# DLR-RB/QUEASARS

Measured on AMD Instinct MI355X. Metric: circuit-evals/sec (EVQE population) at n qubits; achieved HBM GB/s vs roofline, higher is better.
Workload: dtype f64; 1 GPU; 20-qubit EVQE population=64 per GPU, 4 layers, random Ising Hamiltonian (210 terms), fp64 (BASELINE.json configs[1]); n_qubits=20, population_per_gpu=64, layers=4, pauli_terms=210, parallelism=1 GPU

## Files before the change

include/qsv.h:

```cpp
#ifndef QSV_H
#define QSV_H

#include <stddef.h>
#include <stdint.h>

#ifdef __cplusplus
extern "C" {
#endif

typedef struct qsv_handle qsv_t;

enum { QSV_OP_ID = 0, QSV_OP_U = 1, QSV_OP_CU3 = 2 };
enum { QSV_F64 = 0, QSV_F32 = 1 };
enum { QSV_NO_CONTROL = 0xFF };

enum {
    QSV_OK = 0,
    QSV_E_ARG = -1,
    QSV_E_DEVICE = -2,
    QSV_E_STATE = -3,
    QSV_E_UNSUPPORTED = -4
};

typedef struct qsv_op {
// ... 258 lines not shown
int qsv_set_option(qsv_t* h, const char* name, int value);

long long qsv_replayed_pushes(const qsv_t* h);

int qsv_set_profiling(qsv_t* h, int enabled);
int qsv_get_profile(const qsv_t* h, qsv_profile* out);

int qsv_bench_gate(qsv_t* h, int target, int control, double theta, double phi, double lambda, int reps,
                   double* out_ms_per_sweep);

int qsv_bench_ops(qsv_t* h, int n_ops, const qsv_op* ops, int reps, double* out_ms_per_rep, int* out_n_passes);

int qsv_plan_build(int n_qubits, int dtype, int n_ops, const qsv_op* ops, const qsv_plan_config* cfg,
                   uint32_t* out_words, size_t capacity_words, size_t* n_words);

int qsv_split_describe(int n_qubits, int n_ops, const qsv_op* ops, int max_side, uint64_t* mask_a, qsv_op* ops_a,
                       int capacity_a, int* n_ops_a, qsv_op* ops_b, int capacity_b, int* n_ops_b);

#define QSV_SPLIT_MAX_KEYS 8
int qsv_split_describe_reduced(int n_qubits, int n_ops, const qsv_op* ops, int max_side, uint64_t* mask_a, qsv_op* ops_a,
                               int capacity_a, int* n_ops_a, qsv_op* ops_b, int capacity_b, int* n_ops_b,
                               uint32_t* simulated_keys, uint32_t* final_keys, int* key_bits, int* qubits);

const char* qsv_version(void);

#ifdef __cplusplus
}
#endif
#endif
```

queasars_amd/_lib.py:

```python

from __future__ import annotations

import ctypes as C
import os
import threading
from pathlib import Path

import numpy as np

from queasars_amd import _build

QSV_OK, QSV_E_ARG, QSV_E_DEVICE, QSV_E_STATE, QSV_E_UNSUPPORTED = 0, -1, -2, -3, -4
QSV_F64, QSV_F32 = 0, 1


class QsvOp(C.Structure):
    _fields_ = [
        ("kind", C.c_uint8),
        ("target", C.c_uint8),
        ("control", C.c_uint8),
        ("flags", C.c_uint8),
        ("p_theta", C.c_int32),
        ("p_phi", C.c_int32),
        ("p_lambda", C.c_int32),
# ... 247 lines not shown
                                       C.POINTER(C.c_int32), C.POINTER(C.c_int32)]),
    "qsv_adjoint_gradient_circuits": (C.c_int, [_P, C.c_int, _P, _P, _P, _P, _P, _P, _P]),
    "qsv_adjoint_gradient_device": (C.c_int, [_P, C.c_int, _P, C.c_int, _P, _P, _P, _P, C.c_int, _P, _P]),
    "qsv_adjoint_stats": (C.c_int, [_P, C.POINTER(QsvAdjointStats)]),
    "qsv_observables_create": (C.c_int, [_P, C.c_int, _P, _P, _P, _P, _P, C.POINTER(C.c_int)]),
    "qsv_observables_destroy": (C.c_int, [_P, C.c_int]),
    "qsv_eval_observables": (C.c_int, [_P, C.c_int, C.c_int, _P, _P, _P, _P]),
    "qsv_set_option": (C.c_int, [_P, C.c_char_p, C.c_int]),
    "qsv_fitness_table_wait": (C.c_int, [C.c_void_p, C.c_int, C.c_void_p, C.c_int, C.c_int, C.c_int, C.c_int64, C.c_int]),
    "qsv_replayed_pushes": (C.c_longlong, [_P]),
    "qsv_set_profiling": (C.c_int, [_P, C.c_int]),
    "qsv_get_profile": (C.c_int, [_P, C.POINTER(QsvProfile)]),
    "qsv_bench_gate": (C.c_int, [_P, C.c_int, C.c_int, C.c_double, C.c_double, C.c_double, C.c_int, C.POINTER(C.c_double)]),
    "qsv_bench_ops": (C.c_int, [_P, C.c_int, _P, C.c_int, C.POINTER(C.c_double), C.POINTER(C.c_int)]),
    "qsv_split_describe": (
        C.c_int,
        [C.c_int, C.c_int, _P, C.c_int, C.POINTER(C.c_uint64), _P, C.c_int, C.POINTER(C.c_int), _P, C.c_int, C.POINTER(C.c_int)],
    ),
    "qsv_split_describe_reduced": (
        C.c_int,
        [C.c_int, C.c_int, _P, C.c_int, C.POINTER(C.c_uint64), _P, C.c_int, C.POINTER(C.c_int), _P, C.c_int, C.POINTER(C.c_int),
         _P, _P, _P, _P],
    ),
    "qsv_plan_build": (
        C.c_int,
        [C.c_int, C.c_int, C.c_int, _P, C.POINTER(QsvPlanConfig), _P, C.c_size_t, C.POINTER(C.c_size_t)],
    ),
}

_lock = threading.Lock()
_lib = None


class QsvLibraryError(RuntimeError):
    """libqsv is missing or could not be loaded.  There is deliberately no fallback."""


def library_path() -> Path:
    override = os.environ.get("QSV_LIBRARY")
    return Path(override) if override else _build.LIB_PATH


def load(build_if_missing: bool = True) -> C.CDLL:
    global _lib
    with _lock:
        if _lib is not None:
# ... 33 lines not shown
```

queasars_amd/csrc/qsv_api.hip:

```cpp
#include <hip/hip_runtime.h>
#include <immintrin.h>

#include <algorithm>
#include <atomic>
#include <chrono>
#include <cmath>
#include <cstdio>
#include <condition_variable>
#include <cstring>
#include <functional>
#include <memory>
#include <mutex>
#include <string>
#include <thread>
#include <unordered_map>
#include <vector>

#include "../../include/qsv.h"
#include "adjoint.hpp"
#include "gradient.hpp"
#include "value_cache.hpp"
#include "kernels.hpp"
#include "plan.hpp"
#include "split.hpp"
// ... 194 lines not shown
    DeviceBuffer d_factor_big_count;
    uint32_t stream_mode = 0;
    mutable std::mutex mu;
    std::atomic<std::thread::id> batch_owner{};

    int n_terms = 0;
    bool diagonal = false;
    bool has_diag_part = false;
    int n_groups = 0;
    DeviceBuffer d_z, d_cre, d_diag, d_term_partials, d_groups, d_term_odd;
    DeviceBuffer d_order, d_sorted;
    bool order_valid = false;
    int pauli_nb = 0;

    std::unordered_map<int, Circuit> circuits;
    int next_circuit_id = 1;
    std::unordered_map<int, PrefixState> prefixes;
    int next_prefix_id = 1;
    DeviceBuffer d_prefix;
    DeviceBuffer d_sdiag;
    size_t sdiag_used = 0;
    bool side_diag = true;
    bool final_controls = true;
    bool sides_r3 = true;
    size_t prefix_slots = 0;
    std::vector<uint32_t> prefix_free;
    size_t prefix_used = 0;
    std::unordered_map<std::string, int> inline_cache;
    std::unordered_map<int, ObservableSet> obs_sets;
    int next_obs_id = 1;
    DeviceBuffer d_obs_partials, d_obs_values;
    std::unique_ptr<WorkerPool> pool;
    std::mutex pool_mu;

    struct CoalesceRequest {
        int circuit_id = 0;
        const double* params = nullptr;
        int n_params = 0;
        double value = 0.0;
        int rc = QSV_OK;
        std::string err;
        bool done = false;
    };
    std::mutex cq_mu;
    std::condition_variable cq_cv;
    std::vector<CoalesceRequest*> cq;
// ... 397 lines not shown
    }
    out->n_params = n_params;
    out->ops.assign(ops, ops + n_ops);
    out->grad_terms.assign(size_t(n_params), 0);
    (void)gradient_plan(n_ops, ops, n_params, out->grad_terms.data());
    std::vector<AngleSource> angles;
    std::vector<GateIn> gates = gates_of(ops, n_ops, &angles);
    out->n_gates = int(gates.size());
    out->fold = fold;
    try {
        PlanConfig pc = h->cfg;
        pc.fold = pc.fold && fold;
        const bool state_needed = h->n_terms > 0 && !h->diagonal && !h->factor_enabled;
        if (h->split_enabled && !state_needed && pc.fold && h->n > h->geo.k && h->n <= 28) {
            const int side_tile = std::max(h->geo.k, std::min(h->geo.r + 9, int(kMaxTileBits)));
            std::vector<int> limits{h->geo.k};
            if (side_tile > h->geo.k && side_tile < h->n) limits.push_back(side_tile);
            for (int extra = 1; extra <= kSideExtraBits; ++extra) {
                const int limit = std::min(h->geo.k + extra, h->n - 1);
                if (limit > limits.back()) limits.push_back(limit);
            }
            SplitCircuits sc = find_split(h->n, gates, angles, limits, h->split_max_keys);
            if (sc.ok && std::max(sc.n_side[0], sc.n_side[1]) > kSideMaxOwnBits) sc.ok = false;
            if (sc.ok) {
                SplitInfo& sp = out->split;
                std::vector<uint32_t>& w = out->plan.words;
                bool fits = true;
                const bool r3_handle = h->sides_r3 && h->dtype == QSV_F64 && h->geo.k == 12 && h->geo.r == 4 && sc.n_keys <= 3;
                bool try_halves = r3_handle && sc.n_keys >= 1 && std::max(sc.n_side[0], sc.n_side[1]) + sc.n_keys == kFusedLdsRowsBits &&
                                  !getenv("QSV_NO_HALF_SIDES");
                const int most_virtual = std::max(sc.n_side[0], sc.n_side[1]) + sc.n_keys;
                bool try_r3 = try_halves || (r3_handle && (most_virtual <= 12 || (most_virtual == 13 && sc.n_keys >= 1)));
                const size_t words_before = w.size();
                for (bool planned = false; !planned;) {
                planned = true;
                for (int s = 0; s < 2 && fits && planned; ++s) {
                    PlanConfig side = pc;
                    sp.n_virtual[s] = sc.n_side[s] + sc.n_keys;
                    side.tile_bits = std::min(sp.n_virtual[s], side_tile);
                    side.reg_bits = try_r3 ? 3 : h->geo.r;
                    side.compact = false;
                    fits = side.tile_bits > side.reg_bits;
                    if (!fits) break;
                    if (sp.n_virtual[s] <= side.tile_bits) side.lane_bits = 0;
                    if (try_halves && sp.n_virtual[s] == kFusedLdsRowsBits) {
                        side.tile_bits = 12;
                        side.lane_bits = 0;
// ... 73 lines not shown
                    }
                    auto fill = [&](uint32_t* table, uint32_t entries, int first_bit) {
                        table[0] = table[1] = 0;
                        for (uint32_t v = 1; v < entries; ++v) {
                            const uint32_t low = v & (0u - v), rest = v ^ low;
                            const int q = first_bit + __builtin_ctz(low);
                            table[2 * v] = table[2 * rest] | (q < h->n ? colx[size_t(q)] : 0u);
                            table[2 * v + 1] = table[2 * rest + 1] | (q < h->n ? coly[size_t(q)] : 0u);
                        }
                    };
                    fill(blk + kSplitLaneTable, 64, 0);
                    fill(blk + kSplitWaveTable, 1u << wave_bits, 6);
                    fill(blk + kSplitChunkLow, 128, chunk0);
                    fill(blk + kSplitChunkHigh, 128, chunk0 + 7);
                    sp.n_keys = sc.n_keys;
                    sp.ok = true;
                    sp.fused = h->geo.r == 4 && h->geo.k == 12 && sp.n_keys <= 3 && ((sp.outer[0] == 0 && sp.outer[1] == 0) || sp.halves || (sp.side_r == 3 && sp.outer[0] <= 1 && sp.outer[1] <= 1)) &&
                               sp.stats[0].n_passes == 1 && sp.stats[1].n_passes == 1;
                    if (const char* env = getenv("QSV_FUSED_MAX_KEYS")) sp.fused = sp.fused && sp.n_keys <= atoi(env);
                    if (getenv("QSV_SPLIT_DEBUG"))
                        fprintf(stderr, "split: keys %d sides %d+%d virtual %d/%d tiles 2^%d/2^%d passes %d/%d fused %d\n", sp.n_keys, sc.n_side[0],
                                sc.n_side[1], sp.n_virtual[0], sp.n_virtual[1], sp.outer[0], sp.outer[1], sp.stats[0].n_passes,
                                sp.stats[1].n_passes, int(sp.fused));
                    if (sp.fused && h->final_controls) plan_reduced_sides(h, pc, sc, sx, out);
                } else {
                    w.resize(sp.off_side[0] ? sp.off_side[0] : w.size());
                    sp = SplitInfo{};
                }
            }
        }
        if (out->split.ok) {
            out->gates = std::move(gates);
            out->angles = std::move(angles);
        } else {
            const CircuitPlan p = build_ordinary_plan(h, gates, angles, pc);
            out->off_plan = uint32_t(out->plan.words.size());
            out->plan.words.insert(out->plan.words.end(), p.words.begin(), p.words.end());
            out->plan.stats = p.stats;
            out->has_plan = true;
        }
    } catch (const std::exception& e) {
        if (err) *err = std::string("plan: ") + e.what();
        return QSV_E_ARG;
    }
    return QSV_OK;
}

int ensure_plan(qsv_t* h, Circuit& c) {
    if (c.has_plan) return QSV_OK;
    try {
        PlanConfig pc = h->cfg;
// ... 1591 lines not shown
    if (const char* env = getenv("QSV_TILES_PER_BLOCK_LATER")) h->tiles_per_block_later = std::max(1, atoi(env));
    auto bail = [&](hipError_t err, const char* what) {
        std::string msg = std::string(what) + ": " + hipGetErrorString(err);
        qsv_destroy(h);
        return fail(nullptr, QSV_E_DEVICE, msg);
    };
    if ((e = hipStreamCreateWithFlags(&h->stream, hipStreamNonBlocking)) != hipSuccess) return bail(e, "hipStreamCreate");
    h->own_stream = true;
    if (const char* env = getenv("QSV_SPLIT")) h->split_enabled = atoi(env) != 0;
    if (const char* env = getenv("QSV_SPLIT_SAMPLE")) h->split_sampling = atoi(env) != 0;
    if (const char* env = getenv("QSV_FACTOR")) h->factor_enabled = atoi(env) != 0;
    if (getenv("QSV_NO_FUSED_FACTOR")) h->fused_factor = false;
    if (const char* env = getenv("QSV_CHAIN_STREAM")) h->chain_enabled = atoi(env) != 0;
    if (const char* env = getenv("QSV_POLL")) h->poll_results = atoi(env) != 0;
    if (const char* env = getenv("QSV_REPEAT")) h->repeat_enabled = atoi(env) != 0;
    if (const char* env = getenv("QSV_REPLAY")) h->replay_enabled = atoi(env) != 0;
    if (const char* env = getenv("QSV_HOST_TIMING")) h->timing.on = atoi(env) != 0;
    if (const char* env = getenv("QSV_REPEAT_DESCS")) h->repeat_device_descs = atoi(env) != 0;
    if (const char* env = getenv("QSV_FUSED_LDS")) h->fused_lds_table = atoi(env) != 0;
    if (const char* env = getenv("QSV_SIDE_PREPARE")) h->side_prepare = atoi(env) != 0;
    if (const char* env = getenv("QSV_SIDE_DIAG")) h->side_diag = atoi(env) != 0;
    if (const char* env = getenv("QSV_SIDES_R3")) h->sides_r3 = atoi(env) != 0;
    if (const char* env = getenv("QSV_FINAL_CONTROLS")) h->final_controls = atoi(env) != 0;
    {
        int cus = 0;
        if (hipDeviceGetAttribute(&cus, hipDeviceAttributeMultiprocessorCount, device) == hipSuccess && cus > 0) h->n_cus = cus;
        int grid_y = 0;
        if (hipDeviceGetAttribute(&grid_y, hipDeviceAttributeMaxGridDimY, device) == hipSuccess && grid_y > 0)
            h->max_grid_y = h->device_max_grid_y = grid_y;
    }
    {
        int large_bar = 0;
        if (hipDeviceGetAttribute(&large_bar, hipDeviceAttributeIsLargeBar, device) != hipSuccess) large_bar = 0;
        h->bar_ship = false;
        if (const char* env = getenv("QSV_BAR")) h->bar_ship = large_bar != 0 && atoi(env) != 0;
    }
    if (const char* env = getenv("QSV_SPLIT_MAX_KEYS")) h->split_max_keys = std::max(0, std::min(kMaxSplitKeys, atoi(env)));
    h->stream_mode = state_bytes > (size_t(256) << 20) ? uint32_t(kModeStreaming) : 0u;
    if (const char* env = getenv("QSV_STREAMING")) h->stream_mode = atoi(env) ? uint32_t(kModeStreaming) : 0u;
    if (const char* env = getenv("QSV_STREAMS")) h->n_streams = std::max(1, std::min(4, atoi(env)));
    for (int i = 1; i < std::max(2, h->n_streams); ++i) {
        hipStream_t st = nullptr;
        if ((e = hipStreamCreateWithFlags(&st, hipStreamNonBlocking)) != hipSuccess) return bail(e, "hipStreamCreate");
        h->side_streams.push_back(st);
    }
    h->n_lane_streams = int(h->side_streams.size());
// ... 2273 lines not shown
        h->factor_enabled = value != 0;
    } else if (key == "fused_factor") {
        h->fused_factor = value != 0;
    } else if (key == "chain_stream") {
        h->chain_enabled = value != 0;
    } else if (key == "poll_results") {
        h->poll_results = value != 0;
    } else if (key == "repeat_layout") {
        h->repeat_enabled = value != 0;
    } else if (key == "replay_launches") {
        h->replay_enabled = value != 0;
    } else if (key == "split_max_keys") {
        if (value < 0 || value > kMaxSplitKeys) return fail(h, QSV_E_ARG, "split_max_keys must be between 0 and 5");
        h->split_max_keys = value;
    } else if (key == "split_sampling") {
        h->split_sampling = value != 0;
    } else if (key == "fused_lds_table") {
        h->fused_lds_table = value != 0;
    } else if (key == "side_prepare") {
        h->side_prepare = value != 0;
    } else if (key == "final_controls") {
        h->final_controls = value != 0;
        h->epoch += 1;
    } else if (key == "sides_r3") {
        h->sides_r3 = value != 0;
    } else if (key == "side_diag") {
        if (h->side_diag != (value != 0)) {
            QSV_HIP(h, sync_streams(h));
            for (auto& kv : h->circuits) kv.second.uploaded = false;
            h->sdiag_used = 0;
        }
        h->side_diag = value != 0;
    } else if (key == "streams") {
        if (value < 1 || value > h->n_lane_streams + 1) return fail(h, QSV_E_ARG, "streams must be between 1 and the number the handle was created with");
        h->n_streams = value;
    } else if (key == "max_grid_y") {
        if (value < 0 || value > h->device_max_grid_y) return fail(h, QSV_E_ARG, "max_grid_y must be between 0 and the device's largest gridDim.y");
        h->max_grid_y = value ? value : h->device_max_grid_y;
    } else if (key == "gradient_chunk") {
        if (value < 0 || value > (1 << 20)) return fail(h, QSV_E_ARG, "gradient_chunk must be between 0 and 1048576");
        h->grad_chunk = value ? value : kGradientChunkRows;
    } else {
        return fail(h, QSV_E_ARG, "unknown option '" + key + "'");
    }
    return QSV_OK;
}
// ... 110 lines not shown
    if (!sc.ok) return -1;
    *mask_a = sc.mask[0];
    qsv_op* outs[2] = {ops_a, ops_b};
    const int caps[2] = {capacity_a, capacity_b};
    int* counts[2] = {n_ops_a, n_ops_b};
    for (int s = 0; s < 2; ++s) {
        *counts[s] = int(sc.gates[s].size());
        if (!outs[s] || caps[s] < *counts[s]) continue;
        for (size_t i = 0; i < sc.gates[s].size(); ++i) {
            const GateIn& g = sc.gates[s][i];
            const AngleSource& a = sc.angles[s][size_t(g.op)];
            qsv_op o{};
            o.kind = g.control < 0 ? QSV_OP_U : QSV_OP_CU3;
            o.target = uint8_t(g.target);
            o.control = g.control < 0 ? uint8_t(QSV_NO_CONTROL) : uint8_t(g.control);
            o.p_theta = a.p_theta; o.p_phi = a.p_phi; o.p_lambda = a.p_lambda;
            o.theta = a.theta; o.phi = a.phi; o.lambda = a.lambda;
            outs[s][i] = o;
        }
    }
    return sc.n_keys;
}

int qsv_split_describe_reduced(int n_qubits, int n_ops, const qsv_op* ops, int max_side, uint64_t* mask_a, qsv_op* ops_a,
                               int capacity_a, int* n_ops_a, qsv_op* ops_b, int capacity_b, int* n_ops_b,
                               uint32_t* simulated_keys, uint32_t* final_keys, int* key_bits, int* qubits) {
    if (!mask_a || !n_ops_a || !n_ops_b || !simulated_keys || !final_keys || !key_bits || !qubits)
        return fail(nullptr, QSV_E_ARG, "null output") - 100;
    if (n_qubits < 1 || n_qubits > 32) return fail(nullptr, QSV_E_ARG, "n_qubits must be in [1, 32]") - 100;
    if (validate_ops(nullptr, n_qubits, n_ops, ops, 1 << 30)) return QSV_E_ARG - 100;
    std::vector<AngleSource> angles;
    const std::vector<GateIn> gates = gates_of(ops, n_ops, &angles);
    const SplitCircuits sc = find_split(n_qubits, gates, angles, max_side);
    if (!sc.ok) return -1;
    const ReducedSplit rs = reduce_final_controls(sc);
    *mask_a = sc.mask[0];
    qsv_op* outs[2] = {ops_a, ops_b};
    const int caps[2] = {capacity_a, capacity_b};
    int* counts[2] = {n_ops_a, n_ops_b};
    for (int s = 0; s < 2; ++s) {
        simulated_keys[s] = rs.simulated_keys[s];
        final_keys[s] = rs.final_keys[s];
        for (int j = 0; j < QSV_SPLIT_MAX_KEYS; ++j) key_bits[s * QSV_SPLIT_MAX_KEYS + j] = j < kMaxSplitKeys ? rs.key_bit[s][j] : -1;
        std::vector<int> global;
        for (int q = 0; q < n_qubits; ++q)
            if (sc.mask[s] >> q & 1u) global.push_back(q);
        for (int p = 0; p < 32; ++p) qubits[s * 32 + p] = p < sc.n_side[s] ? global[size_t(rs.qubit_of[s][size_t(p)])] : -1;
        *counts[s] = int(rs.gates[s].size());
        if (!outs[s] || caps[s] < *counts[s]) continue;
        for (size_t i = 0; i < rs.gates[s].size(); ++i) {
            const GateIn& g = rs.gates[s][i];
            const AngleSource& a = rs.angles[s][size_t(g.op)];
            qsv_op o{};
            o.kind = g.control < 0 ? QSV_OP_U : QSV_OP_CU3;
            o.target = uint8_t(g.target);
            o.control = g.control < 0 ? uint8_t(QSV_NO_CONTROL) : uint8_t(g.control);
            o.p_theta = a.p_theta; o.p_phi = a.p_phi; o.p_lambda = a.p_lambda;
            o.theta = a.theta; o.phi = a.phi; o.lambda = a.lambda;
            outs[s][i] = o;
        }
    }
    return sc.n_keys;
}

int qsv_plan_build(int n_qubits, int dtype, int n_ops, const qsv_op* ops, const qsv_plan_config* cfg,
                   uint32_t* out_words, size_t capacity_words, size_t* n_words) {
    if (!n_words) return fail(nullptr, QSV_E_ARG, "n_words is null");
    if (dtype != QSV_F64 && dtype != QSV_F32) return fail(nullptr, QSV_E_ARG, "bad dtype");
    if (n_qubits < 1 || n_qubits > 32) return fail(nullptr, QSV_E_ARG, "n_qubits must be in [1, 32]");
    int rc = validate_ops(nullptr, n_qubits, n_ops, ops, 1 << 30);
    if (rc) return rc;
    try {
        PlanConfig pc = resolve_config(cfg, dtype, n_qubits);
        std::vector<AngleSource> angles;
        std::vector<GateIn> gates = gates_of(ops, n_ops, &angles);
        CircuitPlan plan = build_plan(n_qubits, gates, angles, pc);
        *n_words = plan.words.size();
        if (out_words && capacity_words >= plan.words.size())
            std::memcpy(out_words, plan.words.data(), plan.words.size() * 4);
    } catch (const std::exception& e) {
        return fail(nullptr, QSV_E_ARG, e.what());
    }
    return QSV_OK;
}

}
```

queasars_amd/csrc/split.cpp:

```cpp
#include "split.hpp"

#include <algorithm>
#include <array>
#include <cstdlib>
#include <functional>

namespace qsv {

namespace {

struct Key {
    int control;
    std::vector<int> targets;
};

struct UnionFind {
    std::array<int8_t, 64> parent;
    explicit UnionFind(int n) {
        for (int i = 0; i < n; ++i) parent[size_t(i)] = int8_t(i);
    }
    int find(int x) {
        while (parent[size_t(x)] != x) {
            parent[size_t(x)] = parent[size_t(parent[size_t(x)])];
            x = parent[size_t(x)];
        }
        return x;
    }
    void join(int a, int b) { parent[size_t(find(a))] = int8_t(find(b)); }
};

}

SplitCircuits find_split(int n, const std::vector<GateIn>& all_gates, const std::vector<AngleSource>& op_angles,
                         int max_side, int max_keys) {
    return find_split(n, all_gates, op_angles, std::vector<int>{max_side}, max_keys);
}

SplitCircuits find_split(int n, const std::vector<GateIn>& all_gates, const std::vector<AngleSource>& op_angles,
                         const std::vector<int>& max_sides, int max_keys) {
    std::vector<char> open_stage(max_sides.size(), 0);
    bool any_open = false;
    for (size_t s = 0; s < max_sides.size(); ++s) {
        open_stage[s] = !(n > 60 || n <= max_sides[s] || 2 * max_sides[s] < n);
        any_open |= open_stage[s] != 0;
    }
    if (!any_open) return SplitCircuits{};

    std::vector<char> touched(size_t(n), 0);
    std::vector<int> epoch(size_t(n), 0);
    std::vector<int> key_of(all_gates.size(), -1);
    std::vector<char> dropped(all_gates.size(), 0);
    std::vector<Key> keys;
    std::vector<std::pair<int, int>> key_id;
    for (size_t i = 0; i < all_gates.size(); ++i) {
        const GateIn& g = all_gates[i];
        if (g.control >= 0) {
            if (!touched[size_t(g.control)]) {
                dropped[i] = 1;
                continue;
            }
            const std::pair<int, int> id{g.control, epoch[size_t(g.control)]};
            int ki = -1;
            for (size_t j = keys.size(); j-- > 0;)
                if (key_id[j] == id) {
                    ki = int(j);
                    break;
                }
            if (ki < 0) {
                ki = int(keys.size());
                keys.push_back(Key{g.control, {}});
                key_id.push_back(id);
            }
            key_of[i] = ki;
            std::vector<int>& ts = keys[size_t(ki)].targets;
            if (std::find(ts.begin(), ts.end(), g.target) == ts.end()) ts.push_back(g.target);
        }
        touched[size_t(g.target)] = 1;
        epoch[size_t(g.target)] += 1;
    }
    const int nk = int(keys.size());

    std::vector<uint64_t> side_of_stage(max_sides.size(), 0);
    std::vector<char> hit(max_sides.size(), 0);
    size_t first_open = 0;
    while (!open_stage[first_open]) ++first_open;
    bool found = false;
    std::vector<int> without;
    auto try_without = [&]() {
        UnionFind uf(n);
        for (int j = 0; j < nk; ++j) {
            if (std::find(without.begin(), without.end(), j) != without.end()) continue;
            for (int t : keys[size_t(j)].targets) uf.join(keys[size_t(j)].control, t);
        }
        std::array<int8_t, 64> comp_of{};
        std::vector<int> size;
        std::vector<uint64_t> members;
        for (int q = 0; q < n; ++q) {
            const int root = uf.find(q);
            if (root == q) {
                comp_of[size_t(q)] = int8_t(size.size());
                size.push_back(0);
                members.push_back(0);
            }
        }
        for (int q = 0; q < n; ++q) {
            const int c = comp_of[size_t(uf.find(q))];
            size[size_t(c)] += 1;
            members[size_t(c)] |= uint64_t(1) << q;
        }
        const int removed = int(without.size());
        std::vector<uint64_t> choice(size_t(n) + 1, 0);
        std::vector<char> reach(size_t(n) + 1, 0);
        reach[size_t(size[0])] = 1;
        choice[size_t(size[0])] = 1;
        for (size_t c = 1; c < size.size(); ++c)
            for (int s = n - size[c]; s >= 0; --s)
                if (reach[size_t(s)] && !reach[size_t(s + size[c])]) {
                    reach[size_t(s + size[c])] = 1;
                    choice[size_t(s + size[c])] = choice[size_t(s)] | uint64_t(1) << c;
                }
        for (size_t stage = 0; stage < max_sides.size(); ++stage) {
            if (!open_stage[stage] || hit[stage]) continue;
            const int lo = n - max_sides[stage] + removed, hi = max_sides[stage] - removed;
            int best = -1;
            for (int s = lo; s <= hi; ++s)
                if (s >= 0 && s <= n && reach[size_t(s)] && (best < 0 || std::abs(2 * s - n) < std::abs(2 * best - n))) best = s;
            if (best < 0) continue;
            uint64_t side_a = 0;
            for (size_t c = 0; c < size.size(); ++c)
                if (choice[size_t(best)] >> c & 1u) side_a |= members[c];
            side_of_stage[stage] = side_a;
            hit[stage] = 1;
        }
        return hit[first_open] != 0;
    };
    std::vector<std::vector<int>> keys_of_qubit(static_cast<size_t>(n));
    for (int j = 0; j < nk; ++j) {
        keys_of_qubit[size_t(keys[size_t(j)].control)].push_back(j);
        for (int t : keys[size_t(j)].targets) keys_of_qubit[size_t(t)].push_back(j);
    }
    const int n_nodes = n + nk;
    std::vector<int> disc(static_cast<size_t>(n_nodes)), low(static_cast<size_t>(n_nodes)), parent(static_cast<size_t>(n_nodes));
    std::vector<int> next_edge(static_cast<size_t>(n_nodes)), stack;
    std::vector<char> removed(static_cast<size_t>(nk), 0), articulation(static_cast<size_t>(nk), 0);
    auto neighbour = [&](int u, int i) -> int {
        if (u < n) return i < int(keys_of_qubit[size_t(u)].size()) ? n + keys_of_qubit[size_t(u)][size_t(i)] : -1;
        const Key& k = keys[size_t(u - n)];
        if (i == 0) return k.control;
        return i <= int(k.targets.size()) ? k.targets[size_t(i - 1)] : -1;
    };
    auto splitting_keys = [&](std::vector<int>& result) {
        result.clear();
        std::fill(disc.begin(), disc.end(), -1);
        std::fill(articulation.begin(), articulation.end(), 0);
        int clock = 0;
        for (int root = 0; root < n; ++root) {
            if (disc[size_t(root)] >= 0) continue;
            int root_children = 0;
            disc[size_t(root)] = low[size_t(root)] = clock++;
            parent[size_t(root)] = -1;
            next_edge[size_t(root)] = 0;
            stack.assign(1, root);
            while (!stack.empty()) {
                const int u = stack.back();
                const int v = neighbour(u, next_edge[size_t(u)]++);
                if (v < 0) {
                    stack.pop_back();
                    const int p = parent[size_t(u)];
                    if (p >= 0) {
                        low[size_t(p)] = std::min(low[size_t(p)], low[size_t(u)]);
                        if (p != root && p >= n && low[size_t(u)] >= disc[size_t(p)]) articulation[size_t(p - n)] = 1;
                        if (p == root) ++root_children;
                    }
                    continue;
                }
                if (v >= n && removed[size_t(v - n)]) continue;
                if (disc[size_t(v)] < 0) {
                    disc[size_t(v)] = low[size_t(v)] = clock++;
                    parent[size_t(v)] = u;
                    next_edge[size_t(v)] = 0;
                    stack.push_back(v);
                } else if (v != parent[size_t(u)]) {
                    low[size_t(u)] = std::min(low[size_t(u)], disc[size_t(v)]);
                }
            }
            (void)root_children;
        }
        for (int j = 0; j < nk; ++j)
            if (articulation[size_t(j)]) result.push_back(j);
    };
    std::vector<int> last_candidates;
    constexpr int kMaxSweeps = 2000;
    int sweeps = 0;
    std::function<bool(int, int)> choose = [&](int start, int left) {
        if (left == 0) return try_without();
        if (left == 1) {
            if (++sweeps > kMaxSweeps) return false;
            for (int r : without) removed[size_t(r)] = 1;
            splitting_keys(last_candidates);
            for (int r : without) removed[size_t(r)] = 0;
            const std::vector<int> candidates = last_candidates;
            for (int r : candidates) {
                if (r < start) continue;
                without.push_back(r);
                if (try_without()) return true;
                without.pop_back();
            }
            return false;
        }
        for (int r = start; r + left <= nk && sweeps <= kMaxSweeps; ++r) {
            without.push_back(r);
            if (choose(r + 1, left - 1)) return true;
            without.pop_back();
// ... 88 lines not shown
                cut += newly_cut;
                count[s2] += 1;
                side[size_t(v)] = s2;
                if (cut <= bound && count[0] + cut <= largest && count[1] + cut <= largest) descend(depth + 1);
                side[size_t(v)] = -1;
                count[s2] -= 1;
                cut -= newly_cut;
                for (int j : keys_of_qubit[size_t(v)]) --(s2 == 0 ? on_a[size_t(j)] : on_b[size_t(j)]);
            }
        };
        for (bound = 4; bound <= max_keys && !done; ++bound) {
            bool possible = false;
            for (size_t stage = 0; stage < max_sides.size(); ++stage) possible |= open_stage[stage] && 2 * (max_sides[stage] - bound) >= n;
            if (!possible) break;
            nodes = 0;
            descend(0);
            bool got = false;
            for (size_t stage = 0; stage < max_sides.size(); ++stage) got |= hit[stage] != 0;
            if (got) break;
        }
    }
    (void)found;
    for (size_t stage = 0; stage < max_sides.size(); ++stage) {
    if (!hit[stage]) continue;
    const uint64_t side_a = side_of_stage[stage];
    const int max_side = max_sides[stage];
    SplitCircuits out;

    auto side_of = [&](int q) { return int(!(side_a >> q & 1u)); };
    std::vector<int> cut_index(size_t(nk), -1);
    int n_cut = 0;
    for (int j = 0; j < nk; ++j) {
        bool cut = false;
        for (int t : keys[size_t(j)].targets) cut |= side_of(t) != side_of(keys[size_t(j)].control);
        if (cut) cut_index[size_t(j)] = n_cut++;
    }
    out.mask[0] = side_a;
    out.mask[1] = ~side_a & ((uint64_t(1) << n) - 1);
    for (int s = 0; s < 2; ++s) out.n_side[s] = __builtin_popcountll(out.mask[s]);
    if (n_cut > max_keys || out.n_side[0] + n_cut > max_side || out.n_side[1] + n_cut > max_side) continue;
    out.n_keys = n_cut;

    std::vector<int> local(size_t(n), 0);
    {
        int ca = 0, cb = 0;
        for (int q = 0; q < n; ++q) local[size_t(q)] = side_of(q) == 0 ? ca++ : cb++;
    }
    auto fixed = [](int32_t code) { return AngleSource{code, -1, -1, 0.0, 0.0, 0.0}; };
    for (int s = 0; s < 2; ++s) {
        std::vector<GateIn>& vg = out.gates[s];
        std::vector<AngleSource>& va = out.angles[s];
        for (int j = 0; j < n_cut; ++j) {
            va.push_back(fixed(kFixedOnes));
            vg.push_back(GateIn{out.n_side[s] + j, -1, int(va.size()) - 1});
        }
    }
    std::vector<char> projected(size_t(nk), 0);
    for (size_t i = 0; i < all_gates.size(); ++i) {
        if (dropped[i]) continue;
        const GateIn& g = all_gates[i];
        const int st = side_of(g.target);
        const int key = key_of[i] >= 0 ? cut_index[size_t(key_of[i])] : -1;
        if (g.control < 0 || side_of(g.control) == st) {
// ... 12 lines not shown
            out.angles[st].push_back(op_angles[size_t(g.op)]);
            out.gates[st].push_back(GateIn{local[size_t(g.target)], g.control < 0 ? -1 : local[size_t(g.control)],
                                           int(out.angles[st].size()) - 1});
            continue;
        }
        const int sc = 1 - st;
        if (!projected[size_t(key_of[i])]) {
            projected[size_t(key_of[i])] = 1;
            std::vector<GateIn>& vg = out.gates[sc];
            std::vector<AngleSource>& va = out.angles[sc];
            const int c = local[size_t(g.control)], kq = out.n_side[sc] + key;
            va.push_back(fixed(kFixedX));
            vg.push_back(GateIn{c, kq, int(va.size()) - 1});
            va.push_back(fixed(kFixedProj0));
            vg.push_back(GateIn{c, -1, int(va.size()) - 1});
            va.push_back(fixed(kFixedX));
            vg.push_back(GateIn{c, kq, int(va.size()) - 1});
        }
        out.angles[st].push_back(op_angles[size_t(g.op)]);
        out.gates[st].push_back(GateIn{local[size_t(g.target)], out.n_side[st] + key, int(out.angles[st].size()) - 1});
    }
    out.ok = true;
    return out;
    }
    return SplitCircuits{};
}

ReducedSplit reduce_final_controls(const SplitCircuits& full) {
    ReducedSplit out;
    if (!full.ok) return out;
    const int nk = full.n_keys;
    for (int s = 0; s < 2; ++s) {
        const std::vector<GateIn>& fg = full.gates[s];
        const std::vector<AngleSource>& fa = full.angles[s];
        const int ns = full.n_side[s];
        auto code = [&](const GateIn& g) { return fa[size_t(g.op)].p_theta; };
        std::vector<int> control_of(size_t(nk), -1);
        std::vector<char> skip(fg.size(), 0);
        uint32_t finals = 0;
        for (size_t i = 0; i + 2 < fg.size(); ++i) {
            const int j = fg[i].control - ns;
            if (j < 0 || code(fg[i]) != kFixedX || code(fg[i + 1]) != kFixedProj0) continue;
            const int c = fg[i].target;
            bool later = false;
            for (size_t l = i + 3; l < fg.size() && !later; ++l) later = fg[l].target == c;
            if (later) continue;
            finals |= 1u << j;
            control_of[size_t(j)] = c;
// ... 42 lines not shown
```

queasars_amd/csrc/split.hpp:

```cpp
#pragma once

#include <cstdint>
#include <vector>

#include "plan.hpp"

namespace qsv {

constexpr int32_t kFixedProj0 = -2;
constexpr int32_t kFixedOnes = -3;
constexpr int32_t kFixedX = -4;

constexpr int kMaxSplitKeys = 5;

struct SplitCircuits {
    bool ok = false;
    int n_keys = 0;
    int n_side[2] = {0, 0};
    uint64_t mask[2] = {0, 0};
    std::vector<GateIn> gates[2];
    std::vector<AngleSource> angles[2];
};

SplitCircuits find_split(int n_qubits, const std::vector<GateIn>& gates, const std::vector<AngleSource>& op_angles,
                         int max_side, int max_keys = kMaxSplitKeys);
SplitCircuits find_split(int n_qubits, const std::vector<GateIn>& gates, const std::vector<AngleSource>& op_angles,
                         const std::vector<int>& max_sides, int max_keys = kMaxSplitKeys);

struct ReducedSplit {
    bool any = false;
    uint32_t final_keys[2] = {0, 0};
    uint32_t simulated_keys[2] = {0, 0};
    int n_virtual[2] = {0, 0};
    int key_bit[2][kMaxSplitKeys];
    std::vector<int> qubit_of[2];
    std::vector<GateIn> gates[2];
    std::vector<AngleSource> angles[2];
};

ReducedSplit reduce_final_controls(const SplitCircuits& full);

}
```

Baseline: 1.515 million circuit-evals/s.

## Search alternative circuit splits that minimise the larger simulated side

```diff
diff --git a/include/qsv.h b/include/qsv.h
--- a/include/qsv.h
+++ b/include/qsv.h
@@ -304,6 +304,10 @@
                                int capacity_a, int* n_ops_a, qsv_op* ops_b, int capacity_b, int* n_ops_b,
                                uint32_t* simulated_keys, uint32_t* final_keys, int* key_bits, int* qubits);
 
+int qsv_split_describe_chosen(int n_qubits, int n_ops, const qsv_op* ops, int max_side, uint64_t* mask_a, qsv_op* ops_a,
+                              int capacity_a, int* n_ops_a, qsv_op* ops_b, int capacity_b, int* n_ops_b,
+                              uint32_t* simulated_keys, uint32_t* final_keys, int* key_bits, int* qubits);
+
 const char* qsv_version(void);
 
 #ifdef __cplusplus
diff --git a/queasars_amd/_lib.py b/queasars_amd/_lib.py
--- a/queasars_amd/_lib.py
+++ b/queasars_amd/_lib.py
@@ -293,6 +293,11 @@
         [C.c_int, C.c_int, _P, C.c_int, C.POINTER(C.c_uint64), _P, C.c_int, C.POINTER(C.c_int), _P, C.c_int, C.POINTER(C.c_int),
          _P, _P, _P, _P],
     ),
+    "qsv_split_describe_chosen": (
+        C.c_int,
+        [C.c_int, C.c_int, _P, C.c_int, C.POINTER(C.c_uint64), _P, C.c_int, C.POINTER(C.c_int), _P, C.c_int, C.POINTER(C.c_int),
+         _P, _P, _P, _P],
+    ),
     "qsv_plan_build": (
         C.c_int,
         [C.c_int, C.c_int, C.c_int, _P, C.POINTER(QsvPlanConfig), _P, C.c_size_t, C.POINTER(C.c_size_t)],
diff --git a/queasars_amd/csrc/qsv_api.hip b/queasars_amd/csrc/qsv_api.hip
--- a/queasars_amd/csrc/qsv_api.hip
+++ b/queasars_amd/csrc/qsv_api.hip
@@ -240,6 +240,7 @@
     size_t sdiag_used = 0;
     bool side_diag = true;
     bool final_controls = true;
+    bool split_choice = true;
     bool sides_r3 = true;
     size_t prefix_slots = 0;
     std::vector<uint32_t> prefix_free;
@@ -683,7 +684,8 @@
             }
             SplitCircuits sc = find_split(h->n, gates, angles, limits, h->split_max_keys);
             if (sc.ok && std::max(sc.n_side[0], sc.n_side[1]) > kSideMaxOwnBits) sc.ok = false;
-            if (sc.ok) {
+            auto plan_form = [&](const SplitCircuits& sc, bool with_reduced, bool probe_reduced, Circuit* out) -> int {
+                int launched_most = 0;
                 SplitInfo& sp = out->split;
                 std::vector<uint32_t>& w = out->plan.words;
                 bool fits = true;
@@ -803,11 +805,44 @@
                         fprintf(stderr, "split: keys %d sides %d+%d virtual %d/%d tiles 2^%d/2^%d passes %d/%d fused %d\n", sp.n_keys, sc.n_side[0],
                                 sc.n_side[1], sp.n_virtual[0], sp.n_virtual[1], sp.outer[0], sp.outer[1], sp.stats[0].n_passes,
                                 sp.stats[1].n_passes, int(sp.fused));
-                    if (sp.fused && h->final_controls) plan_reduced_sides(h, pc, sc, sx, out);
+                    if (sp.fused) launched_most = std::max(sp.n_virtual[0], sp.n_virtual[1]);
+                    if (sp.fused && with_reduced && (h->final_controls || probe_reduced)) {
+                        const size_t words_full = w.size();
+                        plan_reduced_sides(h, pc, sc, sx, out);
+                        if (out->reduced.ok) launched_most = std::max(out->reduced.n_virtual[0], out->reduced.n_virtual[1]);
+                        if (!h->final_controls) {
+                            w.resize(words_full);
+                            out->reduced = SplitInfo{};
+                            out->reduced_mask[0] = out->reduced_mask[1] = out->reduced_top[0] = out->reduced_top[1] = 0;
+                        }
+                    }
                 } else {
                     w.resize(sp.off_side[0] ? sp.off_side[0] : w.size());
                     sp = SplitInfo{};
                 }
+                return launched_most;
+            };
+            if (sc.ok) {
+                bool replaced = false;
+                if (h->split_choice && h->fused_factor && h->geo.r == 4 && h->geo.k == 12 && sc.n_keys <= 2 && out->plan.words.empty()) {
+                    const SplitChoices choices = split_choices(h->n, gates, angles, sc);
+                    for (const SplitCircuits& form : choices.forms) {
+                        if (std::max(form.n_side[0], form.n_side[1]) > kSideMaxOwnBits) continue;
+                        Circuit trial;
+                        const int most = plan_form(form, choices.reduced, true, &trial);
+                        if (most == 0 || most >= choices.below) continue;
+                        out->plan.words = std::move(trial.plan.words);
+                        out->split = trial.split;
+                        out->reduced = trial.reduced;
+                        for (int xy = 0; xy < 2; ++xy) {
+                            out->reduced_mask[xy] = trial.reduced_mask[xy];
+                            out->reduced_top[xy] = trial.reduced_top[xy];
+                        }
+                        replaced = true;
+                        break;
+                    }
+                }
+                if (!replaced) plan_form(sc, true, false, out);
             }
         }
         if (out->split.ok) {
@@ -2445,6 +2480,7 @@
     if (const char* env = getenv("QSV_SIDE_DIAG")) h->side_diag = atoi(env) != 0;
     if (const char* env = getenv("QSV_SIDES_R3")) h->sides_r3 = atoi(env) != 0;
     if (const char* env = getenv("QSV_FINAL_CONTROLS")) h->final_controls = atoi(env) != 0;
+    if (const char* env = getenv("QSV_SPLIT_CHOICE")) h->split_choice = atoi(env) != 0;
     {
         int cus = 0;
         if (hipDeviceGetAttribute(&cus, hipDeviceAttributeMultiprocessorCount, device) == hipSuccess && cus > 0) h->n_cus = cus;
@@ -4764,6 +4800,8 @@
     } else if (key == "final_controls") {
         h->final_controls = value != 0;
         h->epoch += 1;
+    } else if (key == "split_choice") {
+        h->split_choice = value != 0;
     } else if (key == "sides_r3") {
         h->sides_r3 = value != 0;
     } else if (key == "side_diag") {
@@ -4920,18 +4958,26 @@
     return sc.n_keys;
 }
 
-int qsv_split_describe_reduced(int n_qubits, int n_ops, const qsv_op* ops, int max_side, uint64_t* mask_a, qsv_op* ops_a,
-                               int capacity_a, int* n_ops_a, qsv_op* ops_b, int capacity_b, int* n_ops_b,
-                               uint32_t* simulated_keys, uint32_t* final_keys, int* key_bits, int* qubits) {
+static int describe_reduced(bool chosen, int n_qubits, int n_ops, const qsv_op* ops, int max_side, uint64_t* mask_a, qsv_op* ops_a,
+                            int capacity_a, int* n_ops_a, qsv_op* ops_b, int capacity_b, int* n_ops_b,
+                            uint32_t* simulated_keys, uint32_t* final_keys, int* key_bits, int* qubits) {
     if (!mask_a || !n_ops_a || !n_ops_b || !simulated_keys || !final_keys || !key_bits || !qubits)
         return fail(nullptr, QSV_E_ARG, "null output") - 100;
     if (n_qubits < 1 || n_qubits > 32) return fail(nullptr, QSV_E_ARG, "n_qubits must be in [1, 32]") - 100;
     if (validate_ops(nullptr, n_qubits, n_ops, ops, 1 << 30)) return QSV_E_ARG - 100;
     std::vector<AngleSource> angles;
     const std::vector<GateIn> gates = gates_of(ops, n_ops, &angles);
-    const SplitCircuits sc = find_split(n_qubits, gates, angles, max_side);
+    SplitCircuits sc = find_split(n_qubits, gates, angles, max_side);
     if (!sc.ok) return -1;
-    const ReducedSplit rs = reduce_final_controls(sc);
+    bool reduce = true;
+    if (chosen) {
+        SplitChoices better = split_choices(n_qubits, gates, angles, sc);
+        if (!better.forms.empty()) {
+            sc = std::move(better.forms.front());
+            reduce = better.reduced;
+        }
+    }
+    const ReducedSplit rs = reduce ? reduce_final_controls(sc) : keep_full_form(sc);
     *mask_a = sc.mask[0];
     qsv_op* outs[2] = {ops_a, ops_b};
     const int caps[2] = {capacity_a, capacity_b};
@@ -4961,6 +5007,20 @@
     return sc.n_keys;
 }
 
+int qsv_split_describe_reduced(int n_qubits, int n_ops, const qsv_op* ops, int max_side, uint64_t* mask_a, qsv_op* ops_a,
+                               int capacity_a, int* n_ops_a, qsv_op* ops_b, int capacity_b, int* n_ops_b,
+                               uint32_t* simulated_keys, uint32_t* final_keys, int* key_bits, int* qubits) {
+    return describe_reduced(false, n_qubits, n_ops, ops, max_side, mask_a, ops_a, capacity_a, n_ops_a, ops_b, capacity_b, n_ops_b,
+                            simulated_keys, final_keys, key_bits, qubits);
+}
+
+int qsv_split_describe_chosen(int n_qubits, int n_ops, const qsv_op* ops, int max_side, uint64_t* mask_a, qsv_op* ops_a,
+                              int capacity_a, int* n_ops_a, qsv_op* ops_b, int capacity_b, int* n_ops_b,
+                              uint32_t* simulated_keys, uint32_t* final_keys, int* key_bits, int* qubits) {
+    return describe_reduced(true, n_qubits, n_ops, ops, max_side, mask_a, ops_a, capacity_a, n_ops_a, ops_b, capacity_b, n_ops_b,
+                            simulated_keys, final_keys, key_bits, qubits);
+}
+
 int qsv_plan_build(int n_qubits, int dtype, int n_ops, const qsv_op* ops, const qsv_plan_config* cfg,
                    uint32_t* out_words, size_t capacity_words, size_t* n_words) {
     if (!n_words) return fail(nullptr, QSV_E_ARG, "n_words is null");
diff --git a/queasars_amd/csrc/split.cpp b/queasars_amd/csrc/split.cpp
--- a/queasars_amd/csrc/split.cpp
+++ b/queasars_amd/csrc/split.cpp
@@ -28,6 +28,151 @@
     }
     void join(int a, int b) { parent[size_t(find(a))] = int8_t(find(b)); }
 };
+
+struct KeyAnalysis {
+    std::vector<Key> keys;
+    std::vector<int> key_of;
+    std::vector<char> dropped;
+    std::vector<char> is_final;
+};
+
+KeyAnalysis analyse_keys(int n, const std::vector<GateIn>& all_gates) {
+    KeyAnalysis out;
+    std::vector<char> touched(size_t(n), 0);
+    std::vector<int> epoch(size_t(n), 0);
+    out.key_of.assign(all_gates.size(), -1);
+    out.dropped.assign(all_gates.size(), 0);
+    std::vector<Key>& keys = out.keys;
+    std::vector<std::pair<int, int>> key_id;
+    for (size_t i = 0; i < all_gates.size(); ++i) {
+        const GateIn& g = all_gates[i];
+        if (g.control >= 0) {
+            if (!touched[size_t(g.control)]) {
+                out.dropped[i] = 1;
+                continue;
+            }
+            const std::pair<int, int> id{g.control, epoch[size_t(g.control)]};
+            int ki = -1;
+            for (size_t j = keys.size(); j-- > 0;)
+                if (key_id[j] == id) {
+                    ki = int(j);
+                    break;
+                }
+            if (ki < 0) {
+                ki = int(keys.size());
+                keys.push_back(Key{g.control, {}});
+                key_id.push_back(id);
+            }
+            out.key_of[i] = ki;
+            std::vector<int>& ts = keys[size_t(ki)].targets;
+            if (std::find(ts.begin(), ts.end(), g.target) == ts.end()) ts.push_back(g.target);
+        }
+        touched[size_t(g.target)] = 1;
+        epoch[size_t(g.target)] += 1;
+    }
+    out.is_final.assign(keys.size(), 0);
+    for (size_t j = 0; j < keys.size(); ++j) out.is_final[j] = key_id[j].second == epoch[size_t(key_id[j].first)];
+    return out;
+}
+
+class KeyGraph {
+public:
+    KeyGraph(int n, const std::vector<Key>& keys)
+        : n_(n), nk_(int(keys.size())), keys_(keys), keys_of_qubit(static_cast<size_t>(n)), removed(static_cast<size_t>(nk_), 0),
+          disc_(static_cast<size_t>(n + nk_)), low_(static_cast<size_t>(n + nk_)), parent_(static_cast<size_t>(n + nk_)),
+          next_edge_(static_cast<size_t>(n + nk_)), articulation_(static_cast<size_t>(nk_), 0) {
+        for (int j = 0; j < nk_; ++j) {
+            keys_of_qubit[size_t(keys[size_t(j)].control)].push_back(j);
+            for (int t : keys[size_t(j)].targets) keys_of_qubit[size_t(t)].push_back(j);
+        }
+    }
+    void splitting_keys(std::vector<int>& result) {
+        const int n = n_, nk = nk_;
+        std::vector<int>&disc = disc_, &low = low_, &parent = parent_, &next_edge = next_edge_, &stack = stack_;
+        result.clear();
+        std::fill(disc.begin(), disc.end(), -1);
+        std::fill(articulation_.begin(), articulation_.end(), 0);
+        int clock = 0;
+        for (int root = 0; root < n; ++root) {
+            if (disc[size_t(root)] >= 0) continue;
+            disc[size_t(root)] = low[size_t(root)] = clock++;
+            parent[size_t(root)] = -1;
+            next_edge[size_t(root)] = 0;
+            stack.assign(1, root);
+            while (!stack.empty()) {
+                const int u = stack.back();
+                const int v = neighbour(u, next_edge[size_t(u)]++);
+                if (v < 0) {
+                    stack.pop_back();
+                    const int p = parent[size_t(u)];
+                    if (p >= 0) {
+                        low[size_t(p)] = std::min(low[size_t(p)], low[size_t(u)]);
+                        if (p != root && p >= n && low[size_t(u)] >= disc[size_t(p)]) articulation_[size_t(p - n)] = 1;
+                    }
+                    continue;
+                }
+                if (v >= n && removed[size_t(v - n)]) continue;
+                if (disc[size_t(v)] < 0) {
+                    disc[size_t(v)] = low[size_t(v)] = clock++;
+                    parent[size_t(v)] = u;
+                    next_edge[size_t(v)] = 0;
+                    stack.push_back(v);
+                } else if (v != parent[size_t(u)]) {
+                    low[size_t(u)] = std::min(low[size_t(u)], disc[size_t(v)]);
+                }
+            }
+        }
+        for (int j = 0; j < nk; ++j)
+            if (articulation_[size_t(j)]) result.push_back(j);
+    }
+
+private:
+    int neighbour(int u, int i) const {
+        if (u < n_) return i < int(keys_of_qubit[size_t(u)].size()) ? n_ + keys_of_qubit[size_t(u)][size_t(i)] : -1;
+        const Key& k = keys_[size_t(u - n_)];
+        if (i == 0) return k.control;
+        return i <= int(k.targets.size()) ? k.targets[size_t(i - 1)] : -1;
+    }
+    int n_, nk_;
+    const std::vector<Key>& keys_;
+
+public:
+    std::vector<std::vector<int>> keys_of_qubit;
+    std::vector<char> removed;
+
+private:
+    std::vector<int> disc_, low_, parent_, next_edge_, stack_;
+    std::vector<char> articulation_;
+};
+
+void components_without(int n, const std::vector<Key>& keys, const std::vector<int>& without, std::vector<int>& size,
+                        std::vector<uint64_t>& members) {
+    const int nk = int(keys.size());
+    UnionFind uf(n);
+    for (int j = 0; j < nk; ++j) {
+        if (std::find(without.begin(), without.end(), j) != without.end()) continue;
+        for (int t : keys[size_t(j)].targets) uf.join(keys[size_t(j)].control, t);
+    }
+    std::array<int8_t, 64> comp_of{};
+    size.clear();
+    members.clear();
+    for (int q = 0; q < n; ++q) {
+        const int root = uf.find(q);
+        if (root == q) {
+            comp_of[size_t(q)] = int8_t(size.size());
+            size.push_back(0);
+            members.push_back(0);
+        }
+    }
+    for (int q = 0; q < n; ++q) {
+        const int c = comp_of[size_t(uf.find(q))];
+        size[size_t(c)] += 1;
+        members[size_t(c)] |= uint64_t(1) << q;
+    }
+}
+
+SplitCircuits build_form(int n, const std::vector<GateIn>& all_gates, const std::vector<AngleSource>& op_angles, const KeyAnalysis& ka,
+                         uint64_t side_a, int max_side, int max_keys);
 
 }
 
@@ -46,38 +191,8 @@
     }
     if (!any_open) return SplitCircuits{};
 
-    std::vector<char> touched(size_t(n), 0);
-    std::vector<int> epoch(size_t(n), 0);
-    std::vector<int> key_of(all_gates.size(), -1);
-    std::vector<char> dropped(all_gates.size(), 0);
-    std::vector<Key> keys;
-    std::vector<std::pair<int, int>> key_id;
-    for (size_t i = 0; i < all_gates.size(); ++i) {
-        const GateIn& g = all_gates[i];
-        if (g.control >= 0) {
-            if (!touched[size_t(g.control)]) {
-                dropped[i] = 1;
-                continue;
-            }
-            const std::pair<int, int> id{g.control, epoch[size_t(g.control)]};
-            int ki = -1;
-            for (size_t j = keys.size(); j-- > 0;)
-                if (key_id[j] == id) {
-                    ki = int(j);
-                    break;
-                }
-            if (ki < 0) {
-                ki = int(keys.size());
-                keys.push_back(Key{g.control, {}});
-                key_id.push_back(id);
-            }
-            key_of[i] = ki;
-            std::vector<int>& ts = keys[size_t(ki)].targets;
-            if (std::find(ts.begin(), ts.end(), g.target) == ts.end()) ts.push_back(g.target);
-        }
-        touched[size_t(g.target)] = 1;
-        epoch[size_t(g.target)] += 1;
-    }
+    const KeyAnalysis ka = analyse_keys(n, all_gates);
+    const std::vector<Key>& keys = ka.keys;
     const int nk = int(keys.size());
 
     std::vector<uint64_t> side_of_stage(max_sides.size(), 0);
@@ -87,27 +202,9 @@
     bool found = false;
     std::vector<int> without;
     auto try_without = [&]() {
-        UnionFind uf(n);
-        for (int j = 0; j < nk; ++j) {
-            if (std::find(without.begin(), without.end(), j) != without.end()) continue;
-            for (int t : keys[size_t(j)].targets) uf.join(keys[size_t(j)].control, t);
-        }
-        std::array<int8_t, 64> comp_of{};
         std::vector<int> size;
         std::vector<uint64_t> members;
-        for (int q = 0; q < n; ++q) {
-            const int root = uf.find(q);
-            if (root == q) {
-                comp_of[size_t(q)] = int8_t(size.size());
-                size.push_back(0);
-                members.push_back(0);
-            }
-        }
-        for (int q = 0; q < n; ++q) {
-            const int c = comp_of[size_t(uf.find(q))];
-            size[size_t(c)] += 1;
-            members[size_t(c)] |= uint64_t(1) << q;
-        }
+        components_without(n, keys, without, size, members);
         const int removed = int(without.size());
         std::vector<uint64_t> choice(size_t(n) + 1, 0);
         std::vector<char> reach(size_t(n) + 1, 0);
@@ -134,61 +231,10 @@
         }
         return hit[first_open] != 0;
     };
-    std::vector<std::vector<int>> keys_of_qubit(static_cast<size_t>(n));
-    for (int j = 0; j < nk; ++j) {
-        keys_of_qubit[size_t(keys[size_t(j)].control)].push_back(j);
-        for (int t : keys[size_t(j)].targets) keys_of_qubit[size_t(t)].push_back(j);
-    }
-    const int n_nodes = n + nk;
-    std::vector<int> disc(static_cast<size_t>(n_nodes)), low(static_cast<size_t>(n_nodes)), parent(static_cast<size_t>(n_nodes));
-    std::vector<int> next_edge(static_cast<size_t>(n_nodes)), stack;
-    std::vector<char> removed(static_cast<size_t>(nk), 0), articulation(static_cast<size_t>(nk), 0);
-    auto neighbour = [&](int u, int i) -> int {
-        if (u < n) return i < int(keys_of_qubit[size_t(u)].size()) ? n + keys_of_qubit[size_t(u)][size_t(i)] : -1;
-        const Key& k = keys[size_t(u - n)];
-        if (i == 0) return k.control;
-        return i <= int(k.targets.size()) ? k.targets[size_t(i - 1)] : -1;
-    };
-    auto splitting_keys = [&](std::vector<int>& result) {
-        result.clear();
-        std::fill(disc.begin(), disc.end(), -1);
-        std::fill(articulation.begin(), articulation.end(), 0);
-        int clock = 0;
-        for (int root = 0; root < n; ++root) {
-            if (disc[size_t(root)] >= 0) continue;
-            int root_children = 0;
-            disc[size_t(root)] = low[size_t(root)] = clock++;
-            parent[size_t(root)] = -1;
-            next_edge[size_t(root)] = 0;
-            stack.assign(1, root);
-            while (!stack.empty()) {
-                const int u = stack.back();
-                const int v = neighbour(u, next_edge[size_t(u)]++);
-                if (v < 0) {
-                    stack.pop_back();
-                    const int p = parent[size_t(u)];
-                    if (p >= 0) {
-                        low[size_t(p)] = std::min(low[size_t(p)], low[size_t(u)]);
-                        if (p != root && p >= n && low[size_t(u)] >= disc[size_t(p)]) articulation[size_t(p - n)] = 1;
-                        if (p == root) ++root_children;
-                    }
-                    continue;
-                }
-                if (v >= n && removed[size_t(v - n)]) continue;
-                if (disc[size_t(v)] < 0) {
-                    disc[size_t(v)] = low[size_t(v)] = clock++;
-                    parent[size_t(v)] = u;
-                    next_edge[size_t(v)] = 0;
-                    stack.push_back(v);
-                } else if (v != parent[size_t(u)]) {
-                    low[size_t(u)] = std::min(low[size_t(u)], disc[size_t(v)]);
-                }
-            }
-            (void)root_children;
-        }
-        for (int j = 0; j < nk; ++j)
-            if (articulation[size_t(j)]) result.push_back(j);
-    };
+    KeyGraph graph(n, keys);
+    std::vector<std::vector<int>>& keys_of_qubit = graph.keys_of_qubit;
+    std::vector<char>& removed = graph.removed;
+    auto splitting_keys = [&](std::vector<int>& result) { graph.splitting_keys(result); };
     std::vector<int> last_candidates;
     constexpr int kMaxSweeps = 2000;
     int sweeps = 0;
@@ -323,9 +369,21 @@
     }
     (void)found;
     for (size_t stage = 0; stage < max_sides.size(); ++stage) {
-    if (!hit[stage]) continue;
-    const uint64_t side_a = side_of_stage[stage];
-    const int max_side = max_sides[stage];
+        if (!hit[stage]) continue;
+        SplitCircuits out = build_form(n, all_gates, op_angles, ka, side_of_stage[stage], max_sides[stage], max_keys);
+        if (out.ok) return out;
+    }
+    return SplitCircuits{};
+}
+
+namespace {
+
+SplitCircuits build_form(int n, const std::vector<GateIn>& all_gates, const std::vector<AngleSource>& op_angles, const KeyAnalysis& ka,
+                         uint64_t side_a, int max_side, int max_keys) {
+    const std::vector<Key>& keys = ka.keys;
+    const std::vector<int>& key_of = ka.key_of;
+    const std::vector<char>& dropped = ka.dropped;
+    const int nk = int(keys.size());
     SplitCircuits out;
 
     auto side_of = [&](int q) { return int(!(side_a >> q & 1u)); };
@@ -339,7 +397,7 @@
     out.mask[0] = side_a;
     out.mask[1] = ~side_a & ((uint64_t(1) << n) - 1);
     for (int s = 0; s < 2; ++s) out.n_side[s] = __builtin_popcountll(out.mask[s]);
-    if (n_cut > max_keys || out.n_side[0] + n_cut > max_side || out.n_side[1] + n_cut > max_side) continue;
+    if (n_cut > max_keys || out.n_side[0] + n_cut > max_side || out.n_side[1] + n_cut > max_side) return SplitCircuits{};
     out.n_keys = n_cut;
 
     std::vector<int> local(size_t(n), 0);
@@ -398,8 +456,119 @@
     }
     out.ok = true;
     return out;
-    }
-    return SplitCircuits{};
+}
+
+}
+
+std::vector<SplitCircuits> find_smaller_splits(int n, const std::vector<GateIn>& all_gates, const std::vector<AngleSource>& op_angles,
+                                               int below, int full_most, int max_keys, bool credit_final_controls, int most) {
+    std::vector<SplitCircuits> out;
+    if (n > 60 || n < 2 || 2 * (below - 1) < n || most < 1) return out;
+    const KeyAnalysis ka = analyse_keys(n, all_gates);
+    const std::vector<Key>& keys = ka.keys;
+    const int nk = int(keys.size());
+    max_keys = std::min(max_keys, 2);
+
+    struct Candidate {
+        int cost;
+        uint64_t side_a;
+    };
+    std::vector<Candidate> best;
+    std::vector<int> without, size;
+    std::vector<uint64_t> members;
+    constexpr int kFinals = 3;
+    std::vector<uint64_t> choice((size_t(n) + 1) * kFinals);
+    auto try_without = [&]() {
+        components_without(n, keys, without, size, members);
+        const int removed = int(without.size());
+        std::vector<int> finals(size.size(), 0);
+        int n_finals = 0;
+        for (int j : without)
+            if (credit_final_controls && ka.is_final[size_t(j)])
+                for (size_t c = 0; c < size.size(); ++c)
+                    if (members[c] >> keys[size_t(j)].control & 1u) {
+                        finals[c] += 1;
+                        n_finals += 1;
+                    }
+        std::fill(choice.begin(), choice.end(), 0);
+        choice[size_t(size[0] * kFinals + finals[0])] = 1;
+        for (size_t c = 1; c < size.size(); ++c)
+            for (int s = n - size[c]; s >= 0; --s)
+                for (int f = n_finals - finals[c]; f >= 0; --f) {
+                    const size_t from = size_t(s * kFinals + f), to = size_t((s + size[c]) * kFinals + f + finals[c]);
+                    if (choice[from] && !choice[to]) choice[to] = choice[from] | uint64_t(1) << c;
+                }
+        int pick = -1, cost = 0, spread = 0;
+        for (int s = 1; s < n; ++s)
+            for (int f = 0; f <= n_finals; ++f) {
+                if (!choice[size_t(s * kFinals + f)] || std::max(s, n - s) + removed > full_most) continue;
+                const int larger = std::max(s + removed - f, n - s + removed - (n_finals - f));
+                if (pick < 0 || larger < cost || (larger == cost && std::abs(2 * s - n) < spread)) {
+                    pick = s * kFinals + f;
+                    cost = larger;
+                    spread = std::abs(2 * s - n);
+                }
+            }
+        if (pick < 0 || cost >= below || (int(best.size()) == most && cost >= best.back().cost)) return;
+        uint64_t side_a = 0;
+        for (size_t c = 0; c < size.size(); ++c)
+            if (choice[size_t(pick)] >> c & 1u) side_a |= members[c];
+        for (const Candidate& b : best)
+            if (b.side_a == side_a) return;
+        size_t at = best.size();
+        while (at > 0 && best[at - 1].cost > cost) --at;
+        best.insert(best.begin() + long(at), Candidate{cost, side_a});
+        if (int(best.size()) > most) best.pop_back();
+    };
+    KeyGraph graph(n, keys);
+    std::vector<int> splitting;
+    try_without();
+    for (int first = -1; first < nk && max_keys >= 1; ++first) {
+        if (first >= 0 && max_keys < 2) break;
+        without.clear();
+        if (first >= 0) {
+            without.push_back(first);
+            graph.removed[size_t(first)] = 1;
+        }
+        graph.splitting_keys(splitting);
+        if (first >= 0) graph.removed[size_t(first)] = 0;
+        for (int last : splitting) {
+            if (last <= first) continue;
+            without.push_back(last);
+            try_without();
+            without.pop_back();
+        }
+    }
+    for (const Candidate& b : best) {
+        SplitCircuits form = build_form(n, all_gates, op_angles, ka, b.side_a, n, max_keys);
+        if (form.ok) out.push_back(std::move(form));
+    }
+    return out;
+}
+
+SplitChoices split_choices(int n, const std::vector<GateIn>& gates, const std::vector<AngleSource>& op_angles, const SplitCircuits& today) {
+    SplitChoices out;
+    if (!today.ok || today.n_keys > 2) return out;
+    const ReducedSplit rs = reduce_final_controls(today);
+    out.reduced = rs.any;
+    out.below = std::max(rs.n_virtual[0], rs.n_virtual[1]);
+    const int full_most = std::max(today.n_side[0], today.n_side[1]) + today.n_keys;
+    out.forms = find_smaller_splits(n, gates, op_angles, out.below, full_most, std::min(today.n_keys + 1, 2), out.reduced, 2);
+    return out;
+}
+
+ReducedSplit keep_full_form(const SplitCircuits& full) {
+    ReducedSplit out;
+    if (!full.ok) return out;
+    for (int s = 0; s < 2; ++s) {
+        out.simulated_keys[s] = (1u << full.n_keys) - 1u;
+        out.n_virtual[s] = full.n_side[s] + full.n_keys;
+        for (int j = 0; j < kMaxSplitKeys; ++j) out.key_bit[s][j] = j < full.n_keys ? full.n_side[s] + j : -1;
+        for (int q = 0; q < full.n_side[s]; ++q) out.qubit_of[s].push_back(q);
+        out.gates[s] = full.gates[s];
+        out.angles[s] = full.angles[s];
+    }
+    return out;
 }
 
 ReducedSplit reduce_final_controls(const SplitCircuits& full) {
diff --git a/queasars_amd/csrc/split.hpp b/queasars_amd/csrc/split.hpp
--- a/queasars_amd/csrc/split.hpp
+++ b/queasars_amd/csrc/split.hpp
@@ -27,6 +27,9 @@
 SplitCircuits find_split(int n_qubits, const std::vector<GateIn>& gates, const std::vector<AngleSource>& op_angles,
                          const std::vector<int>& max_sides, int max_keys = kMaxSplitKeys);
 
+std::vector<SplitCircuits> find_smaller_splits(int n_qubits, const std::vector<GateIn>& gates, const std::vector<AngleSource>& op_angles,
+                                               int below, int full_most, int max_keys, bool credit_final_controls, int most);
+
 struct ReducedSplit {
     bool any = false;
     uint32_t final_keys[2] = {0, 0};
@@ -40,4 +43,13 @@
 
 ReducedSplit reduce_final_controls(const SplitCircuits& full);
 
+ReducedSplit keep_full_form(const SplitCircuits& full);
+
+struct SplitChoices {
+    int below = 0;
+    bool reduced = false;
+    std::vector<SplitCircuits> forms;
+};
+SplitChoices split_choices(int n_qubits, const std::vector<GateIn>& gates, const std::vector<AngleSource>& op_angles, const SplitCircuits& today);
+
 }
```

After: 1.496 million circuit-evals/s. -1.3%, worse.
